# Zejun-Yang/AniPortrait

Measured on NVIDIA H100. Metric: denoised frames/sec @512x512 L=16 steps=25, higher is better.
Workload: dtype fp16

## Files before the change

### aniportrait_b200/csrc/ap_attention.cu

```cuda
#include <stdio.h>
#include <stdlib.h>

#include "ap_host.h"
#include "ap_ptx.cuh"
#include "ap_wgmma.cuh"

namespace ap {

__device__ __forceinline__ float fast_exp2(float x) {
  float y;
  asm("ex2.approx.ftz.f32 %0, %1;" : "=f"(y) : "f"(x));
  return y;
}

struct AttnParams {
  int n_frames, tokens, heads, head_dim;
  int bank_tokens;
  int first_bank_frame;
  int frames_per_bank;
  int m_tiles;
  int num_units;
  float scale_log2;
  __half* out;
  long long ldo;
};

template <int DPAD, int BN>
struct AttnCfg {
  static constexpr int SLABS = DPAD / 64;
  static constexpr int Q_BYTES = 128 * DPAD * 2;
  static constexpr int K_BYTES = BN * DPAD * 2;
  static constexpr int KV_STAGE = 2 * K_BYTES;
  static constexpr int BUDGET = 227 * 1024 - 1024 - 256 - Q_BYTES;
  static constexpr int STAGES_RAW = BUDGET / KV_STAGE;
  static constexpr int STAGES = STAGES_RAW > 4 ? 4 : STAGES_RAW;
  static constexpr int SMEM_BYTES = Q_BYTES + STAGES * KV_STAGE + 1024 + 256;
  static_assert(STAGES >= 2, "need at least a double-buffered K/V ring");
  static_assert(DPAD % 64 == 0 && DPAD <= 192 && (BN == 64 || BN == 128), "tile config");
};

template <int DPAD, int BN>
__global__ void __launch_bounds__(384, 1)
attention_kernel(const __grid_constant__ CUtensorMap tmQ, const __grid_constant__ CUtensorMap tmK,
                 const __grid_constant__ CUtensorMap tmV, const __grid_constant__ CUtensorMap tmBK,
                 const __grid_constant__ CUtensorMap tmBV, const AttnParams p) {
  using Cfg = AttnCfg<DPAD, BN>;
  constexpr int ST = Cfg::STAGES;
  griddep_launch_dependents();
  extern __shared__ uint8_t smem_raw[];
  uint8_t* smem = reinterpret_cast<uint8_t*>((reinterpret_cast<uintptr_t>(smem_raw) + 1023) & ~uintptr_t(1023));
  uint8_t* smem_q = smem;
  uint8_t* smem_kv = smem_q + Cfg::Q_BYTES;
  uint64_t* bars = reinterpret_cast<uint64_t*>(smem_kv + ST * Cfg::KV_STAGE);
  uint64_t* q_full = bars + 0;
  uint64_t* q_empty = bars + 1;
  uint64_t* k_full = bars + 2;
  uint64_t* v_full = k_full + ST;
  uint64_t* kv_empty = v_full + ST;

  const int warp = threadIdx.x >> 5;
  const int lane = threadIdx.x & 31;

  if (warp == 0 && lane == 0) {
    tma_prefetch_desc(&tmQ);
    tma_prefetch_desc(&tmK);
    tma_prefetch_desc(&tmV);
    mbar_init(q_full, 1);
    mbar_init(q_empty, 8);
    for (int s = 0; s < ST; ++s) {
      mbar_init(&k_full[s], 1);
      mbar_init(&v_full[s], 1);
      mbar_init(&kv_empty[s], 8);
    }
    fence_mbar_init();
  }
  __syncthreads();
  griddep_wait();

  const int own_tiles = (p.tokens + BN - 1) / BN;
  const int bank_tiles = (p.bank_tokens + BN - 1) / BN;
  const int units_per_frame = p.heads * p.m_tiles;

  auto decode = [&](int unit, int& frame, int& head, int& m_tile, int& T) {
    const int fk = unit / units_per_frame;
    const int rem = unit % units_per_frame;
    frame = (fk + p.first_bank_frame) % p.n_frames;
    head = rem / p.m_tiles;
    m_tile = rem % p.m_tiles;
    const bool has_bank = p.bank_tokens > 0 && frame >= p.first_bank_frame;
    T = own_tiles + (has_bank ? bank_tiles : 0);
  };

  if (warp < 4) {
    setmaxnreg_dec<40>();
    if (warp == 0 && lane == 0) {
      uint32_t g = 0;
      uint32_t uc = 0;
      for (int unit = blockIdx.x; unit < p.num_units; unit += gridDim.x, ++uc) {
        int frame, head, m_tile, T;
        decode(unit, frame, head, m_tile, T);
        mbar_wait_quiet(q_empty, (uc & 1) ^ 1);
        mbar_arrive_expect_tx(q_full, Cfg::Q_BYTES);
#pragma unroll
        for (int s = 0; s < Cfg::SLABS; ++s)
          tma_load_2d(&tmQ, q_full, smem_q + s * (128 * 128), head * DPAD + s * 64, frame * p.tokens + m_tile * 128);
        const int bank_idx = (frame - p.first_bank_frame) / p.frames_per_bank;
        for (int j = 0; j < T; ++j, ++g) {
          const int stage = g % ST;
          const uint32_t ph = (g / ST) & 1;
          mbar_wait_quiet(&kv_empty[stage], ph ^ 1);
          const bool own = j < own_tiles;
          const CUtensorMap* mk = own ? &tmK : &tmBK;
          const CUtensorMap* mv = own ? &tmV : &tmBV;
          const int row = own ? frame * p.tokens + j * BN : bank_idx * p.bank_tokens + (j - own_tiles) * BN;
          uint8_t* kd = smem_kv + stage * Cfg::KV_STAGE;
          uint8_t* vd = kd + Cfg::K_BYTES;
          mbar_arrive_expect_tx(&k_full[stage], Cfg::K_BYTES);
#pragma unroll
          for (int s = 0; s < Cfg::SLABS; ++s)
            tma_load_2d(mk, &k_full[stage], kd + s * (BN * 128), head * DPAD + s * 64, row);
          mbar_arrive_expect_tx(&v_full[stage], Cfg::K_BYTES);
#pragma unroll
          for (int s = 0; s < Cfg::SLABS; ++s)
            tma_load_2d(mv, &v_full[stage], vd + s * (BN * 128), head * DPAD + s * 64, row);
        }
      }
    }
    return;
  }

  setmaxnreg_inc<232>();
  const int wg = (warp >> 2) - 1;
  const int wq = warp & 3;
  const int qd = lane & 3;
  const uint32_t q_base = smem_u32(smem_q) + wg * (64 * 128);
  uint32_t g = 0, uc = 0;
  for (int unit = blockIdx.x; unit < p.num_units; unit += gridDim.x, ++uc) {
    int frame, head, m_tile, T;
    decode(unit, frame, head, m_tile, T);
    float o[DPAD / 2];
#pragma unroll
    for (int i = 0; i < DPAD / 2; ++i) o[i] = 0.f;
    float m_run[2] = {-INFINITY, -INFINITY}, l_run[2] = {0.f, 0.f};
    mbar_wait_quiet(q_full, uc & 1);
    for (int j = 0; j < T; ++j, ++g) {
      const int stage = g % ST;
      const uint32_t ph = (g / ST) & 1;
      const uint32_t k_addr = smem_u32(smem_kv + stage * Cfg::KV_STAGE);
      const uint32_t v_addr = k_addr + Cfg::K_BYTES;
      float s[BN / 2];
      mbar_wait_quiet(&k_full[stage], ph);
      wgmma_fence();
#pragma unroll
      for (int kk = 0; kk < DPAD / 16; ++kk)
        wgmma_ss<BN>(s, wgmma_desc_k_sw128(q_base + (kk / 4) * (128 * 128) + (kk % 4) * 32),
                     wgmma_desc_k_sw128(k_addr + (kk / 4) * (BN * 128) + (kk % 4) * 32), kk != 0);
      wgmma_commit();
      wgmma_wait<0>();
      reg_fence<BN / 2>(s);
      if (j == T - 1) {
        __syncwarp();
        if (lane == 0) mbar_arrive(q_empty);
      }

      const bool own = j < own_tiles;
      const int jj = own ? j : j - own_tiles;
      const int ntok = own ? p.tokens : p.bank_tokens;
      const int valid = min(BN, ntok - jj * BN);
      if (valid != BN) {
#pragma unroll
        for (int i = 0; i < BN / 8; ++i)
#pragma unroll
          for (int e = 0; e < 2; ++e)
            if (8 * i + 2 * qd + e >= valid) {
              s[4 * i + e] = -INFINITY;
              s[4 * i + 2 + e] = -INFINITY;
            }
      }
      float mx[2] = {s[0], s[2]};
#pragma unroll
      for (int i = 0; i < BN / 8; ++i) {
        mx[0] = fmaxf(mx[0], fmaxf(s[4 * i], s[4 * i + 1]));
        mx[1] = fmaxf(mx[1], fmaxf(s[4 * i + 2], s[4 * i + 3]));
      }
      float alpha[2];
#pragma unroll
      for (int r = 0; r < 2; ++r) {
        mx[r] = fmaxf(mx[r], __shfl_xor_sync(0xffffffffu, mx[r], 1));
        mx[r] = fmaxf(mx[r], __shfl_xor_sync(0xffffffffu, mx[r], 2));
        const float m_new = fmaxf(m_run[r], mx[r] * p.scale_log2);
        alpha[r] = fast_exp2(m_run[r] - m_new);
        m_run[r] = m_new;
        l_run[r] *= alpha[r];
      }
#pragma unroll
      for (int i = 0; i < DPAD / 8; ++i) {
        o[4 * i] *= alpha[0]; o[4 * i + 1] *= alpha[0];
        o[4 * i + 2] *= alpha[1]; o[4 * i + 3] *= alpha[1];
      }
      uint32_t pk[BN / 4];
#pragma unroll
      for (int i = 0; i < BN / 8; ++i) {
        const float p0 = fast_exp2(fmaf(s[4 * i], p.scale_log2, -m_run[0]));
        const float p1 = fast_exp2(fmaf(s[4 * i + 1], p.scale_log2, -m_run[0]));
        const float p2 = fast_exp2(fmaf(s[4 * i + 2], p.scale_log2, -m_run[1]));
        const float p3 = fast_exp2(fmaf(s[4 * i + 3], p.scale_log2, -m_run[1]));
        l_run[0] += p0 + p1;
        l_run[1] += p2 + p3;
        const __half2 h01 = __floats2half2_rn(p0, p1), h23 = __floats2half2_rn(p2, p3);
        pk[2 * i] = *reinterpret_cast<const uint32_t*>(&h01);
        pk[2 * i + 1] = *reinterpret_cast<const uint32_t*>(&h23);
      }
      mbar_wait_quiet(&v_full[stage], ph);
      wgmma_fence();
#pragma unroll
      for (int kk = 0; kk < BN / 16; ++kk)
        wgmma_rs_tb<DPAD>(o, pk + 4 * kk, wgmma_desc_mn_sw128(v_addr + kk * (16 * 128), BN * 128), 1);
      wgmma_commit();
      wgmma_wait<0>();
      reg_fence<DPAD / 2>(o);
      __syncwarp();
      if (lane == 0) mbar_arrive(&kv_empty[stage]);
    }
#pragma unroll
    for (int r = 0; r < 2; ++r) {
      l_run[r] += __shfl_xor_sync(0xffffffffu, l_run[r], 1);
      l_run[r] += __shfl_xor_sync(0xffffffffu, l_run[r], 2);
    }
#pragma unroll
    for (int r = 0; r < 2; ++r) {
      const float inv_l = 1.f / l_run[r];
      const int q_idx = m_tile * 128 + wg * 64 + wq * 16 + (lane >> 2) + 8 * r;
      if (q_idx < p.tokens) {
        __half* dst = p.out + ((long long)frame * p.tokens + q_idx) * p.ldo + head * p.head_dim;
#pragma unroll
        for (int i = 0; i < DPAD / 8; ++i)
          if (8 * i + 2 * qd < p.head_dim)
            *reinterpret_cast<__half2*>(dst + 8 * i + 2 * qd) =
                __floats2half2_rn(o[4 * i + 2 * r] * inv_l, o[4 * i + 2 * r + 1] * inv_l);
      }
    }
  }
}

template <int DPAD, int BN>
static int launch_attention(const CUtensorMap* maps, const AttnParams& p, cudaStream_t stream) {
  using Cfg = AttnCfg<DPAD, BN>;
  static bool attr_set = false;
  if (!attr_set) {
    AP_CHECK_CUDA(cudaFuncSetAttribute(attention_kernel<DPAD, BN>, cudaFuncAttributeMaxDynamicSharedMemorySize,
                                       Cfg::SMEM_BYTES));
    attr_set = true;
  }
  const int grid = p.num_units < num_sms() ? p.num_units : num_sms();
  AP_LAUNCH((attention_kernel<DPAD, BN>), grid, 384, Cfg::SMEM_BYTES, stream, maps[0], maps[1], maps[2], maps[3], maps[4], p);
  AP_CHECK_CUDA(cudaGetLastError());
  return AP_OK;
}

}

using namespace ap;

extern "C" int ap_attention_f16(const void* q, const void* k, const void* v, long long ld_qkv, const void* bank_k,
                                const void* bank_v, long long ld_bank, int bank_tokens, int n_banks, int n_frames,
                                int tokens, int heads, int head_dim, int dpad, int first_bank_frame,
                                int frames_per_bank, float scale, void* out, long long ldo, void* stream) {
  AP_REQUIRE(q && k && v && out, "attention: null pointer");
  AP_REQUIRE(dpad == 64 || dpad == 128 || dpad == 192, "attention: dpad must be 64/128/192 (got %d)", dpad);
  AP_REQUIRE(head_dim % 8 == 0 && head_dim <= dpad, "attention: head_dim %d must be a multiple of 8 and <= dpad", head_dim);
  AP_REQUIRE(ld_qkv % 8 == 0 && ldo % 8 == 0, "attention: leading dims must be multiples of 8 elements");
  AP_REQUIRE((reinterpret_cast<uintptr_t>(out) & 3) == 0, "attention: out must be 4-byte aligned");
  AP_REQUIRE(n_frames > 0 && tokens > 0 && heads > 0, "attention: bad shape");
  const bool has_bank = bank_k != nullptr && bank_tokens > 0;
  AP_REQUIRE(!has_bank || (bank_v && frames_per_bank > 0 && first_bank_frame >= 0 && n_banks > 0),
             "attention: bad bank arguments");
  const int bn = dpad == 192 ? 64 : 128;
  AttnParams p{};
  p.n_frames = n_frames;
  p.tokens = tokens;
  p.heads = heads;
  p.head_dim = head_dim;
  p.bank_tokens = has_bank ? bank_tokens : 0;
  p.first_bank_frame = has_bank ? first_bank_frame : 0;
  p.frames_per_bank = has_bank ? frames_per_bank : 1;
  p.m_tiles = (tokens + 127) / 128;
  p.num_units = n_frames * heads * p.m_tiles;
  p.scale_log2 = scale * 1.4426950408889634f;
  p.out = (__half*)out;
  p.ldo = ldo;
  if (has_bank) {
    const int max_bank = (n_frames - 1 - first_bank_frame) / frames_per_bank;
    AP_REQUIRE(first_bank_frame >= n_frames || max_bank < n_banks, "attention: bank index out of range");
  }

  CUtensorMap maps[5];
  const uint64_t cols = (uint64_t)heads * dpad;
  auto mk = [&](CUtensorMap* tm, const void* base, uint64_t rows, long long ld, uint32_t box_rows) -> int {
    const uint64_t dims[2] = {cols, rows};
    const uint64_t strides[1] = {(uint64_t)ld * 2};
    const uint32_t box[2] = {64, box_rows};
    return encode_tmap(tm, base, 2, dims, strides, box, true);
  };
  int rc;
  const uint64_t rows = (uint64_t)n_frames * tokens;
  if ((rc = mk(&maps[0], q, rows, ld_qkv, 128))) return rc;
  if ((rc = mk(&maps[1], k, rows, ld_qkv, bn))) return rc;
  if ((rc = mk(&maps[2], v, rows, ld_qkv, bn))) return rc;
  if (has_bank) {
    const uint64_t brows = (uint64_t)n_banks * bank_tokens;
    if ((rc = mk(&maps[3], bank_k, brows, ld_bank, bn))) return rc;
    if ((rc = mk(&maps[4], bank_v, brows, ld_bank, bn))) return rc;
  } else {
    maps[3] = maps[1];
    maps[4] = maps[2];
  }
  cudaStream_t st = (cudaStream_t)stream;
  if (dpad == 64) return launch_attention<64, 128>(maps, p, st);
  if (dpad == 128) return launch_attention<128, 128>(maps, p, st);
  return launch_attention<192, 64>(maps, p, st);
}
```

### aniportrait_b200/csrc/ap_ptx.cuh

```cuda
#pragma once
#include <cuda.h>
#include <cuda_fp16.h>
#include <cuda_runtime.h>
#include <stdint.h>
#include <stdio.h>

namespace ap {

__device__ __forceinline__ void griddep_launch_dependents() { asm volatile("griddepcontrol.launch_dependents;" ::: "memory"); }
__device__ __forceinline__ void griddep_wait() { asm volatile("griddepcontrol.wait;" ::: "memory"); }

__device__ __forceinline__ float gelu_erf(float x) {
  const float z = fminf(fabsf(x) * 0.70710678118654752f, 4.3f);
  float q = fmaf(1.686094986e-05f, z, -4.376256625e-04f);
  q = fmaf(q, z, 4.960034474e-03f);
  q = fmaf(q, z, -3.321249048e-02f);
  q = fmaf(q, z, 1.515097036e-01f);
  q = fmaf(q, z, 9.176268788e-01f);
  q = fmaf(q, z, 1.627959694e+00f);
  float e;
  asm("ex2.approx.ftz.f32 %0, %1;" : "=f"(e) : "f"(-q * z));
  return fmaxf(x, 0.f) - z * 0.70710678118654752f * e;
}

__device__ __forceinline__ float quick_gelu(float x) {
  float e, r;
  asm("ex2.approx.ftz.f32 %0, %1;" : "=f"(e) : "f"(x * -2.4554669595930157f));
  asm("rcp.approx.ftz.f32 %0, %1;" : "=f"(r) : "f"(1.f + e));
  return x * r;
}

__device__ __forceinline__ uint32_t smem_u32(const void* p) {
  return static_cast<uint32_t>(__cvta_generic_to_shared(p));
}

__device__ __forceinline__ uint32_t elect_one() {
  uint32_t pred = 0;
  asm volatile(
      "{\n\t"
      ".reg .pred P1;\n\t"
      "elect.sync _|P1, 0xffffffff;\n\t"
      "selp.u32 %0, 1, 0, P1;\n\t"
      "}\n"
      : "=r"(pred));
  return pred;
}

__device__ __forceinline__ void mbar_init(uint64_t* bar, uint32_t count) {
  asm volatile("mbarrier.init.shared::cta.b64 [%0], %1;" ::"r"(smem_u32(bar)), "r"(count) : "memory");
}
__device__ __forceinline__ void fence_mbar_init() {
  asm volatile("fence.mbarrier_init.release.cluster;" ::: "memory");
}
__device__ __forceinline__ void fence_proxy_async_smem() {
  asm volatile("fence.proxy.async.shared::cta;" ::: "memory");
}
__device__ __forceinline__ void mbar_arrive_expect_tx(uint64_t* bar, uint32_t bytes) {
  asm volatile("mbarrier.arrive.expect_tx.shared::cta.b64 _, [%0], %1;" ::"r"(smem_u32(bar)), "r"(bytes)
               : "memory");
}
__device__ __forceinline__ void mbar_arrive(uint64_t* bar) {
  asm volatile("mbarrier.arrive.shared::cta.b64 _, [%0];" ::"r"(smem_u32(bar)) : "memory");
}
__device__ __forceinline__ uint32_t mbar_try_wait(uint64_t* bar, uint32_t parity) {
  uint32_t done;
  asm volatile(
      "{\n\t"
      ".reg .pred P1;\n\t"
      "mbarrier.try_wait.parity.shared::cta.b64 P1, [%1], %2;\n\t"
      "selp.u32 %0, 1, 0, P1;\n\t"
      "}\n"
      : "=r"(done)
      : "r"(smem_u32(bar)), "r"(parity)
      : "memory");
  return done;
}
#ifndef AP_MBAR_TIMEOUT_CYCLES
#define AP_MBAR_TIMEOUT_CYCLES (8000000000ll)
#endif
__device__ __forceinline__ void mbar_wait(uint64_t* bar, uint32_t parity) {
  if (mbar_try_wait(bar, parity)) return;
  long long t0 = clock64();
  while (!mbar_try_wait(bar, parity)) {
    if (clock64() - t0 > AP_MBAR_TIMEOUT_CYCLES) {
      printf("ap: mbarrier timeout block=(%d,%d) thread=%d bar=0x%x parity=%u\n", blockIdx.x, blockIdx.y, threadIdx.x,
             smem_u32(bar), parity);
      __trap();
    }
  }
}

__device__ __forceinline__ void mbar_wait_quiet(uint64_t* bar, uint32_t parity) {
  if (mbar_try_wait(bar, parity)) return;
  long long t0 = clock64();
  while (!mbar_try_wait(bar, parity))
    if (clock64() - t0 > AP_MBAR_TIMEOUT_CYCLES) __trap();
}

__device__ __forceinline__ void tma_prefetch_desc(const CUtensorMap* m) {
  asm volatile("prefetch.tensormap [%0];" ::"l"(reinterpret_cast<uint64_t>(m)) : "memory");
}
__device__ __forceinline__ void tma_load_2d(const CUtensorMap* m, uint64_t* bar, void* dst, int c0, int c1) {
  asm volatile(
      "cp.async.bulk.tensor.2d.shared::cluster.global.mbarrier::complete_tx::bytes [%0], [%1, {%3, %4}], [%2];" ::"r"(
          smem_u32(dst)),
      "l"(reinterpret_cast<uint64_t>(m)), "r"(smem_u32(bar)), "r"(c0), "r"(c1)
      : "memory");
}
__device__ __forceinline__ void tma_load_3d(const CUtensorMap* m, uint64_t* bar, void* dst, int c0, int c1, int c2) {
  asm volatile(
      "cp.async.bulk.tensor.3d.shared::cluster.global.mbarrier::complete_tx::bytes [%0], [%1, {%3, %4, %5}], [%2];" ::
          "r"(smem_u32(dst)),
      "l"(reinterpret_cast<uint64_t>(m)), "r"(smem_u32(bar)), "r"(c0), "r"(c1), "r"(c2)
      : "memory");
}
__device__ __forceinline__ void tma_load_4d(const CUtensorMap* m, uint64_t* bar, void* dst, int c0, int c1, int c2,
                                            int c3) {
  asm volatile(
      "cp.async.bulk.tensor.4d.shared::cluster.global.mbarrier::complete_tx::bytes [%0], [%1, {%3, %4, %5, %6}], "
      "[%2];" ::"r"(smem_u32(dst)),
      "l"(reinterpret_cast<uint64_t>(m)), "r"(smem_u32(bar)), "r"(c0), "r"(c1), "r"(c2), "r"(c3)
      : "memory");
}
__device__ __forceinline__ void tma_load_5d(const CUtensorMap* m, uint64_t* bar, void* dst, int c0, int c1, int c2,
                                            int c3, int c4) {
  asm volatile(
      "cp.async.bulk.tensor.5d.shared::cluster.global.mbarrier::complete_tx::bytes [%0], [%1, {%3, %4, %5, %6, %7}], "
      "[%2];" ::"r"(smem_u32(dst)),
      "l"(reinterpret_cast<uint64_t>(m)), "r"(smem_u32(bar)), "r"(c0), "r"(c1), "r"(c2), "r"(c3), "r"(c4)
      : "memory");
}

__device__ __forceinline__ void tma_store_2d(const CUtensorMap* m, const void* src, int c0, int c1) {
  asm volatile("cp.async.bulk.tensor.2d.global.shared::cta.bulk_group [%0, {%2, %3}], [%1];" ::"l"(
                   reinterpret_cast<uint64_t>(m)),
               "r"(smem_u32(src)), "r"(c0), "r"(c1)
               : "memory");
}
__device__ __forceinline__ void tma_store_4d(const CUtensorMap* m, const void* src, int c0, int c1, int c2, int c3) {
  asm volatile("cp.async.bulk.tensor.4d.global.shared::cta.bulk_group [%0, {%2, %3, %4, %5}], [%1];" ::"l"(
                   reinterpret_cast<uint64_t>(m)),
               "r"(smem_u32(src)), "r"(c0), "r"(c1), "r"(c2), "r"(c3)
               : "memory");
}
__device__ __forceinline__ void tma_store_commit() { asm volatile("cp.async.bulk.commit_group;" ::: "memory"); }
template <int N>
__device__ __forceinline__ void tma_store_wait_read() {
  asm volatile("cp.async.bulk.wait_group.read %0;" ::"n"(N) : "memory");
}
template <int N>
__device__ __forceinline__ void tma_store_wait_all() {
  asm volatile("cp.async.bulk.wait_group %0;" ::"n"(N) : "memory");
}

__device__ __forceinline__ void wgmma_fence() { asm volatile("wgmma.fence.sync.aligned;" ::: "memory"); }
__device__ __forceinline__ void wgmma_commit() { asm volatile("wgmma.commit_group.sync.aligned;" ::: "memory"); }
template <int N>
__device__ __forceinline__ void wgmma_wait() {
  asm volatile("wgmma.wait_group.sync.aligned %0;" ::"n"(N) : "memory");
}
template <int N>
__device__ __forceinline__ void reg_fence(float* r) {
#pragma unroll
  for (int i = 0; i < N; ++i) asm volatile("" : "+f"(r[i])::"memory");
}
template <uint32_t kRegs>
__device__ __forceinline__ void setmaxnreg_inc() { asm volatile("setmaxnreg.inc.sync.aligned.u32 %0;" ::"n"(kRegs)); }
template <uint32_t kRegs>
__device__ __forceinline__ void setmaxnreg_dec() { asm volatile("setmaxnreg.dec.sync.aligned.u32 %0;" ::"n"(kRegs)); }

__device__ __forceinline__ uint64_t wgmma_desc_k_sw128(uint32_t smem_addr) {
  uint64_t d = 0;
  d |= static_cast<uint64_t>((smem_addr >> 4) & 0x3FFF);
  d |= static_cast<uint64_t>(1) << 16;
  d |= static_cast<uint64_t>(1024 >> 4) << 32;
  d |= static_cast<uint64_t>(1) << 62;
  return d;
}
__device__ __forceinline__ uint64_t wgmma_desc_mn_sw128(uint32_t smem_addr, uint32_t lbo_bytes) {
  uint64_t d = 0;
  d |= static_cast<uint64_t>((smem_addr >> 4) & 0x3FFF);
  d |= static_cast<uint64_t>((lbo_bytes >> 4) & 0x3FFF) << 16;
  d |= static_cast<uint64_t>(1024 >> 4) << 32;
  d |= static_cast<uint64_t>(1) << 62;
  return d;
}

__device__ __forceinline__ void named_bar_sync(uint32_t id, uint32_t nthreads) {
  asm volatile("bar.sync %0, %1;" ::"r"(id), "r"(nthreads) : "memory");
}

}
```

### aniportrait_b200/csrc/ap_wgmma.cuh

```cuda
#pragma once
#include <stdint.h>

namespace ap {

template <int N>
__device__ __forceinline__ void wgmma_ss(float* d, uint64_t da, uint64_t db, uint32_t scale_d);
template <int N>
__device__ __forceinline__ void wgmma_rs_tb(float* d, const uint32_t* a, uint64_t db, uint32_t scale_d);

template <>
__device__ __forceinline__ void wgmma_ss<32>(float* d, uint64_t da, uint64_t db, uint32_t scale_d) {
  asm volatile(
      "{\n\t.reg .pred p;\n\tsetp.ne.b32 p, %18, 0;\n\t"
      "wgmma.mma_async.sync.aligned.m64n32k16.f32.f16.f16 {%0, %1, %2, %3, %4, %5, %6, %7, %8, %9, %10, %11, %12, %13, %14, %15}, %16, %17, p, 1, 1, 0, 0;\n\t}\n"
      : "+f"(d[0]), "+f"(d[1]), "+f"(d[2]), "+f"(d[3]), "+f"(d[4]), "+f"(d[5]), "+f"(d[6]), "+f"(d[7]), "+f"(d[8]), "+f"(d[9]), "+f"(d[10]), "+f"(d[11]), "+f"(d[12]), "+f"(d[13]), "+f"(d[14]), "+f"(d[15])
      : "l"(da), "l"(db), "r"(scale_d));
}
template <>
__device__ __forceinline__ void wgmma_ss<64>(float* d, uint64_t da, uint64_t db, uint32_t scale_d) {
  asm volatile(
      "{\n\t.reg .pred p;\n\tsetp.ne.b32 p, %34, 0;\n\t"
      "wgmma.mma_async.sync.aligned.m64n64k16.f32.f16.f16 {%0, %1, %2, %3, %4, %5, %6, %7, %8, %9, %10, %11, %12, %13, %14, %15, %16, %17, %18, %19, %20, %21, %22, %23, %24, %25, %26, %27, %28, %29, %30, %31}, %32, %33, p, 1, 1, 0, 0;\n\t}\n"
      : "+f"(d[0]), "+f"(d[1]), "+f"(d[2]), "+f"(d[3]), "+f"(d[4]), "+f"(d[5]), "+f"(d[6]), "+f"(d[7]), "+f"(d[8]), "+f"(d[9]), "+f"(d[10]), "+f"(d[11]), "+f"(d[12]), "+f"(d[13]), "+f"(d[14]), "+f"(d[15]), "+f"(d[16]), "+f"(d[17]), "+f"(d[18]), "+f"(d[19]), "+f"(d[20]), "+f"(d[21]), "+f"(d[22]), "+f"(d[23]), "+f"(d[24]), "+f"(d[25]), "+f"(d[26]), "+f"(d[27]), "+f"(d[28]), "+f"(d[29]), "+f"(d[30]), "+f"(d[31])
      : "l"(da), "l"(db), "r"(scale_d));
}
template <>
__device__ __forceinline__ void wgmma_ss<128>(float* d, uint64_t da, uint64_t db, uint32_t scale_d) {
  asm volatile(
      "{\n\t.reg .pred p;\n\tsetp.ne.b32 p, %66, 0;\n\t"
      "wgmma.mma_async.sync.aligned.m64n128k16.f32.f16.f16 {%0, %1, %2, %3, %4, %5, %6, %7, %8, %9, %10, %11, %12, %13, %14, %15, %16, %17, %18, %19, %20, %21, %22, %23, %24, %25, %26, %27, %28, %29, %30, %31, %32, %33, %34, %35, %36, %37, %38, %39, %40, %41, %42, %43, %44, %45, %46, %47, %48, %49, %50, %51, %52, %53, %54, %55, %56, %57, %58, %59, %60, %61, %62, %63}, %64, %65, p, 1, 1, 0, 0;\n\t}\n"
      : "+f"(d[0]), "+f"(d[1]), "+f"(d[2]), "+f"(d[3]), "+f"(d[4]), "+f"(d[5]), "+f"(d[6]), "+f"(d[7]), "+f"(d[8]), "+f"(d[9]), "+f"(d[10]), "+f"(d[11]), "+f"(d[12]), "+f"(d[13]), "+f"(d[14]), "+f"(d[15]), "+f"(d[16]), "+f"(d[17]), "+f"(d[18]), "+f"(d[19]), "+f"(d[20]), "+f"(d[21]), "+f"(d[22]), "+f"(d[23]), "+f"(d[24]), "+f"(d[25]), "+f"(d[26]), "+f"(d[27]), "+f"(d[28]), "+f"(d[29]), "+f"(d[30]), "+f"(d[31]), "+f"(d[32]), "+f"(d[33]), "+f"(d[34]), "+f"(d[35]), "+f"(d[36]), "+f"(d[37]), "+f"(d[38]), "+f"(d[39]), "+f"(d[40]), "+f"(d[41]), "+f"(d[42]), "+f"(d[43]), "+f"(d[44]), "+f"(d[45]), "+f"(d[46]), "+f"(d[47]), "+f"(d[48]), "+f"(d[49]), "+f"(d[50]), "+f"(d[51]), "+f"(d[52]), "+f"(d[53]), "+f"(d[54]), "+f"(d[55]), "+f"(d[56]), "+f"(d[57]), "+f"(d[58]), "+f"(d[59]), "+f"(d[60]), "+f"(d[61]), "+f"(d[62]), "+f"(d[63])
      : "l"(da), "l"(db), "r"(scale_d));
}
template <>
__device__ __forceinline__ void wgmma_ss<160>(float* d, uint64_t da, uint64_t db, uint32_t scale_d) {
  asm volatile(
      "{\n\t.reg .pred p;\n\tsetp.ne.b32 p, %82, 0;\n\t"
      "wgmma.mma_async.sync.aligned.m64n160k16.f32.f16.f16 {%0, %1, %2, %3, %4, %5, %6, %7, %8, %9, %10, %11, %12, %13, %14, %15, %16, %17, %18, %19, %20, %21, %22, %23, %24, %25, %26, %27, %28, %29, %30, %31, %32, %33, %34, %35, %36, %37, %38, %39, %40, %41, %42, %43, %44, %45, %46, %47, %48, %49, %50, %51, %52, %53, %54, %55, %56, %57, %58, %59, %60, %61, %62, %63, %64, %65, %66, %67, %68, %69, %70, %71, %72, %73, %74, %75, %76, %77, %78, %79}, %80, %81, p, 1, 1, 0, 0;\n\t}\n"
      : "+f"(d[0]), "+f"(d[1]), "+f"(d[2]), "+f"(d[3]), "+f"(d[4]), "+f"(d[5]), "+f"(d[6]), "+f"(d[7]), "+f"(d[8]), "+f"(d[9]), "+f"(d[10]), "+f"(d[11]), "+f"(d[12]), "+f"(d[13]), "+f"(d[14]), "+f"(d[15]), "+f"(d[16]), "+f"(d[17]), "+f"(d[18]), "+f"(d[19]), "+f"(d[20]), "+f"(d[21]), "+f"(d[22]), "+f"(d[23]), "+f"(d[24]), "+f"(d[25]), "+f"(d[26]), "+f"(d[27]), "+f"(d[28]), "+f"(d[29]), "+f"(d[30]), "+f"(d[31]), "+f"(d[32]), "+f"(d[33]), "+f"(d[34]), "+f"(d[35]), "+f"(d[36]), "+f"(d[37]), "+f"(d[38]), "+f"(d[39]), "+f"(d[40]), "+f"(d[41]), "+f"(d[42]), "+f"(d[43]), "+f"(d[44]), "+f"(d[45]), "+f"(d[46]), "+f"(d[47]), "+f"(d[48]), "+f"(d[49]), "+f"(d[50]), "+f"(d[51]), "+f"(d[52]), "+f"(d[53]), "+f"(d[54]), "+f"(d[55]), "+f"(d[56]), "+f"(d[57]), "+f"(d[58]), "+f"(d[59]), "+f"(d[60]), "+f"(d[61]), "+f"(d[62]), "+f"(d[63]), "+f"(d[64]), "+f"(d[65]), "+f"(d[66]), "+f"(d[67]), "+f"(d[68]), "+f"(d[69]), "+f"(d[70]), "+f"(d[71]), "+f"(d[72]), "+f"(d[73]), "+f"(d[74]), "+f"(d[75]), "+f"(d[76]), "+f"(d[77]), "+f"(d[78]), "+f"(d[79])
      : "l"(da), "l"(db), "r"(scale_d));
}
template <>
__device__ __forceinline__ void wgmma_ss<256>(float* d, uint64_t da, uint64_t db, uint32_t scale_d) {
  asm volatile(
      "{\n\t.reg .pred p;\n\tsetp.ne.b32 p, %130, 0;\n\t"
      "wgmma.mma_async.sync.aligned.m64n256k16.f32.f16.f16 {%0, %1, %2, %3, %4, %5, %6, %7, %8, %9, %10, %11, %12, %13, %14, %15, %16, %17, %18, %19, %20, %21, %22, %23, %24, %25, %26, %27, %28, %29, %30, %31, %32, %33, %34, %35, %36, %37, %38, %39, %40, %41, %42, %43, %44, %45, %46, %47, %48, %49, %50, %51, %52, %53, %54, %55, %56, %57, %58, %59, %60, %61, %62, %63, %64, %65, %66, %67, %68, %69, %70, %71, %72, %73, %74, %75, %76, %77, %78, %79, %80, %81, %82, %83, %84, %85, %86, %87, %88, %89, %90, %91, %92, %93, %94, %95, %96, %97, %98, %99, %100, %101, %102, %103, %104, %105, %106, %107, %108, %109, %110, %111, %112, %113, %114, %115, %116, %117, %118, %119, %120, %121, %122, %123, %124, %125, %126, %127}, %128, %129, p, 1, 1, 0, 0;\n\t}\n"
      : "+f"(d[0]), "+f"(d[1]), "+f"(d[2]), "+f"(d[3]), "+f"(d[4]), "+f"(d[5]), "+f"(d[6]), "+f"(d[7]), "+f"(d[8]), "+f"(d[9]), "+f"(d[10]), "+f"(d[11]), "+f"(d[12]), "+f"(d[13]), "+f"(d[14]), "+f"(d[15]), "+f"(d[16]), "+f"(d[17]), "+f"(d[18]), "+f"(d[19]), "+f"(d[20]), "+f"(d[21]), "+f"(d[22]), "+f"(d[23]), "+f"(d[24]), "+f"(d[25]), "+f"(d[26]), "+f"(d[27]), "+f"(d[28]), "+f"(d[29]), "+f"(d[30]), "+f"(d[31]), "+f"(d[32]), "+f"(d[33]), "+f"(d[34]), "+f"(d[35]), "+f"(d[36]), "+f"(d[37]), "+f"(d[38]), "+f"(d[39]), "+f"(d[40]), "+f"(d[41]), "+f"(d[42]), "+f"(d[43]), "+f"(d[44]), "+f"(d[45]), "+f"(d[46]), "+f"(d[47]), "+f"(d[48]), "+f"(d[49]), "+f"(d[50]), "+f"(d[51]), "+f"(d[52]), "+f"(d[53]), "+f"(d[54]), "+f"(d[55]), "+f"(d[56]), "+f"(d[57]), "+f"(d[58]), "+f"(d[59]), "+f"(d[60]), "+f"(d[61]), "+f"(d[62]), "+f"(d[63]), "+f"(d[64]), "+f"(d[65]), "+f"(d[66]), "+f"(d[67]), "+f"(d[68]), "+f"(d[69]), "+f"(d[70]), "+f"(d[71]), "+f"(d[72]), "+f"(d[73]), "+f"(d[74]), "+f"(d[75]), "+f"(d[76]), "+f"(d[77]), "+f"(d[78]), "+f"(d[79]), "+f"(d[80]), "+f"(d[81]), "+f"(d[82]), "+f"(d[83]), "+f"(d[84]), "+f"(d[85]), "+f"(d[86]), "+f"(d[87]), "+f"(d[88]), "+f"(d[89]), "+f"(d[90]), "+f"(d[91]), "+f"(d[92]), "+f"(d[93]), "+f"(d[94]), "+f"(d[95]), "+f"(d[96]), "+f"(d[97]), "+f"(d[98]), "+f"(d[99]), "+f"(d[100]), "+f"(d[101]), "+f"(d[102]), "+f"(d[103]), "+f"(d[104]), "+f"(d[105]), "+f"(d[106]), "+f"(d[107]), "+f"(d[108]), "+f"(d[109]), "+f"(d[110]), "+f"(d[111]), "+f"(d[112]), "+f"(d[113]), "+f"(d[114]), "+f"(d[115]), "+f"(d[116]), "+f"(d[117]), "+f"(d[118]), "+f"(d[119]), "+f"(d[120]), "+f"(d[121]), "+f"(d[122]), "+f"(d[123]), "+f"(d[124]), "+f"(d[125]), "+f"(d[126]), "+f"(d[127])
      : "l"(da), "l"(db), "r"(scale_d));
}
template <>
__device__ __forceinline__ void wgmma_rs_tb<64>(float* d, const uint32_t* a, uint64_t db, uint32_t scale_d) {
  asm volatile(
      "{\n\t.reg .pred p;\n\tsetp.ne.b32 p, %37, 0;\n\t"
      "wgmma.mma_async.sync.aligned.m64n64k16.f32.f16.f16 {%0, %1, %2, %3, %4, %5, %6, %7, %8, %9, %10, %11, %12, %13, %14, %15, %16, %17, %18, %19, %20, %21, %22, %23, %24, %25, %26, %27, %28, %29, %30, %31}, {%32, %33, %34, %35}, %36, p, 1, 1, 1;\n\t}\n"
      : "+f"(d[0]), "+f"(d[1]), "+f"(d[2]), "+f"(d[3]), "+f"(d[4]), "+f"(d[5]), "+f"(d[6]), "+f"(d[7]), "+f"(d[8]), "+f"(d[9]), "+f"(d[10]), "+f"(d[11]), "+f"(d[12]), "+f"(d[13]), "+f"(d[14]), "+f"(d[15]), "+f"(d[16]), "+f"(d[17]), "+f"(d[18]), "+f"(d[19]), "+f"(d[20]), "+f"(d[21]), "+f"(d[22]), "+f"(d[23]), "+f"(d[24]), "+f"(d[25]), "+f"(d[26]), "+f"(d[27]), "+f"(d[28]), "+f"(d[29]), "+f"(d[30]), "+f"(d[31])
      : "r"(a[0]), "r"(a[1]), "r"(a[2]), "r"(a[3]), "l"(db), "r"(scale_d));
}
template <>
__device__ __forceinline__ void wgmma_rs_tb<128>(float* d, const uint32_t* a, uint64_t db, uint32_t scale_d) {
  asm volatile(
      "{\n\t.reg .pred p;\n\tsetp.ne.b32 p, %69, 0;\n\t"
      "wgmma.mma_async.sync.aligned.m64n128k16.f32.f16.f16 {%0, %1, %2, %3, %4, %5, %6, %7, %8, %9, %10, %11, %12, %13, %14, %15, %16, %17, %18, %19, %20, %21, %22, %23, %24, %25, %26, %27, %28, %29, %30, %31, %32, %33, %34, %35, %36, %37, %38, %39, %40, %41, %42, %43, %44, %45, %46, %47, %48, %49, %50, %51, %52, %53, %54, %55, %56, %57, %58, %59, %60, %61, %62, %63}, {%64, %65, %66, %67}, %68, p, 1, 1, 1;\n\t}\n"
      : "+f"(d[0]), "+f"(d[1]), "+f"(d[2]), "+f"(d[3]), "+f"(d[4]), "+f"(d[5]), "+f"(d[6]), "+f"(d[7]), "+f"(d[8]), "+f"(d[9]), "+f"(d[10]), "+f"(d[11]), "+f"(d[12]), "+f"(d[13]), "+f"(d[14]), "+f"(d[15]), "+f"(d[16]), "+f"(d[17]), "+f"(d[18]), "+f"(d[19]), "+f"(d[20]), "+f"(d[21]), "+f"(d[22]), "+f"(d[23]), "+f"(d[24]), "+f"(d[25]), "+f"(d[26]), "+f"(d[27]), "+f"(d[28]), "+f"(d[29]), "+f"(d[30]), "+f"(d[31]), "+f"(d[32]), "+f"(d[33]), "+f"(d[34]), "+f"(d[35]), "+f"(d[36]), "+f"(d[37]), "+f"(d[38]), "+f"(d[39]), "+f"(d[40]), "+f"(d[41]), "+f"(d[42]), "+f"(d[43]), "+f"(d[44]), "+f"(d[45]), "+f"(d[46]), "+f"(d[47]), "+f"(d[48]), "+f"(d[49]), "+f"(d[50]), "+f"(d[51]), "+f"(d[52]), "+f"(d[53]), "+f"(d[54]), "+f"(d[55]), "+f"(d[56]), "+f"(d[57]), "+f"(d[58]), "+f"(d[59]), "+f"(d[60]), "+f"(d[61]), "+f"(d[62]), "+f"(d[63])
      : "r"(a[0]), "r"(a[1]), "r"(a[2]), "r"(a[3]), "l"(db), "r"(scale_d));
}
template <>
__device__ __forceinline__ void wgmma_rs_tb<192>(float* d, const uint32_t* a, uint64_t db, uint32_t scale_d) {
  asm volatile(
      "{\n\t.reg .pred p;\n\tsetp.ne.b32 p, %101, 0;\n\t"
      "wgmma.mma_async.sync.aligned.m64n192k16.f32.f16.f16 {%0, %1, %2, %3, %4, %5, %6, %7, %8, %9, %10, %11, %12, %13, %14, %15, %16, %17, %18, %19, %20, %21, %22, %23, %24, %25, %26, %27, %28, %29, %30, %31, %32, %33, %34, %35, %36, %37, %38, %39, %40, %41, %42, %43, %44, %45, %46, %47, %48, %49, %50, %51, %52, %53, %54, %55, %56, %57, %58, %59, %60, %61, %62, %63, %64, %65, %66, %67, %68, %69, %70, %71, %72, %73, %74, %75, %76, %77, %78, %79, %80, %81, %82, %83, %84, %85, %86, %87, %88, %89, %90, %91, %92, %93, %94, %95}, {%96, %97, %98, %99}, %100, p, 1, 1, 1;\n\t}\n"
      : "+f"(d[0]), "+f"(d[1]), "+f"(d[2]), "+f"(d[3]), "+f"(d[4]), "+f"(d[5]), "+f"(d[6]), "+f"(d[7]), "+f"(d[8]), "+f"(d[9]), "+f"(d[10]), "+f"(d[11]), "+f"(d[12]), "+f"(d[13]), "+f"(d[14]), "+f"(d[15]), "+f"(d[16]), "+f"(d[17]), "+f"(d[18]), "+f"(d[19]), "+f"(d[20]), "+f"(d[21]), "+f"(d[22]), "+f"(d[23]), "+f"(d[24]), "+f"(d[25]), "+f"(d[26]), "+f"(d[27]), "+f"(d[28]), "+f"(d[29]), "+f"(d[30]), "+f"(d[31]), "+f"(d[32]), "+f"(d[33]), "+f"(d[34]), "+f"(d[35]), "+f"(d[36]), "+f"(d[37]), "+f"(d[38]), "+f"(d[39]), "+f"(d[40]), "+f"(d[41]), "+f"(d[42]), "+f"(d[43]), "+f"(d[44]), "+f"(d[45]), "+f"(d[46]), "+f"(d[47]), "+f"(d[48]), "+f"(d[49]), "+f"(d[50]), "+f"(d[51]), "+f"(d[52]), "+f"(d[53]), "+f"(d[54]), "+f"(d[55]), "+f"(d[56]), "+f"(d[57]), "+f"(d[58]), "+f"(d[59]), "+f"(d[60]), "+f"(d[61]), "+f"(d[62]), "+f"(d[63]), "+f"(d[64]), "+f"(d[65]), "+f"(d[66]), "+f"(d[67]), "+f"(d[68]), "+f"(d[69]), "+f"(d[70]), "+f"(d[71]), "+f"(d[72]), "+f"(d[73]), "+f"(d[74]), "+f"(d[75]), "+f"(d[76]), "+f"(d[77]), "+f"(d[78]), "+f"(d[79]), "+f"(d[80]), "+f"(d[81]), "+f"(d[82]), "+f"(d[83]), "+f"(d[84]), "+f"(d[85]), "+f"(d[86]), "+f"(d[87]), "+f"(d[88]), "+f"(d[89]), "+f"(d[90]), "+f"(d[91]), "+f"(d[92]), "+f"(d[93]), "+f"(d[94]), "+f"(d[95])
      : "r"(a[0]), "r"(a[1]), "r"(a[2]), "r"(a[3]), "l"(db), "r"(scale_d));
}

}
```

Before: 5.681.

## Ping-pong warpgroups, overlap PV with next QK, trim MMA width to head dim

The two consumer warpgroups now take turns issuing tensor-core work through named barriers, so one warpgroup's softmax overlaps the other's MMAs. Within each warpgroup, the P·V MMA for tile j and the Q·K MMA for tile j+1 go out in a single batch, which cuts wgmma wait points. The P·V output width and the QK k-steps are templated on the real head dim (40/80/88/160), so the padded columns are no longer computed. The row-max uses a tree reduction, and the K/V ring may grow to 6 stages. In exchange, the barrier bookkeeping for the last unit and for T==1 is more intricate, and there is a deadlock or correctness risk if the turn barriers fall out of sync.

Measured after the change: 5.724 (median of 6 runs). About the same (+0.8%).

```diff
diff --git a/aniportrait_b200/csrc/ap_attention.cu b/aniportrait_b200/csrc/ap_attention.cu
--- a/aniportrait_b200/csrc/ap_attention.cu
+++ b/aniportrait_b200/csrc/ap_attention.cu
@@ -33,19 +33,21 @@
   static constexpr int KV_STAGE = 2 * K_BYTES;
   static constexpr int BUDGET = 227 * 1024 - 1024 - 256 - Q_BYTES;
   static constexpr int STAGES_RAW = BUDGET / KV_STAGE;
-  static constexpr int STAGES = STAGES_RAW > 4 ? 4 : STAGES_RAW;
+  static constexpr int STAGES = STAGES_RAW > 6 ? 6 : STAGES_RAW;
   static constexpr int SMEM_BYTES = Q_BYTES + STAGES * KV_STAGE + 1024 + 256;
   static_assert(STAGES >= 2, "need at least a double-buffered K/V ring");
   static_assert(DPAD % 64 == 0 && DPAD <= 192 && (BN == 64 || BN == 128), "tile config");
 };
 
-template <int DPAD, int BN>
+template <int DPAD, int BN, int NV>
 __global__ void __launch_bounds__(384, 1)
 attention_kernel(const __grid_constant__ CUtensorMap tmQ, const __grid_constant__ CUtensorMap tmK,
                  const __grid_constant__ CUtensorMap tmV, const __grid_constant__ CUtensorMap tmBK,
                  const __grid_constant__ CUtensorMap tmBV, const AttnParams p) {
   using Cfg = AttnCfg<DPAD, BN>;
   constexpr int ST = Cfg::STAGES;
+  constexpr int KSTEPS = (NV + 15) / 16;
+  static_assert(NV % 8 == 0 && NV <= DPAD, "MMA width");
   griddep_launch_dependents();
   extern __shared__ uint8_t smem_raw[];
   uint8_t* smem = reinterpret_cast<uint8_t*>((reinterpret_cast<uintptr_t>(smem_raw) + 1023) & ~uintptr_t(1023));
@@ -134,35 +136,42 @@
   const int wq = warp & 3;
   const int qd = lane & 3;
   const uint32_t q_base = smem_u32(smem_q) + wg * (64 * 128);
+  constexpr uint32_t TURN_BAR = 1;
+  if (wg == 1) named_bar_arrive(TURN_BAR + 0, 256);
   uint32_t g = 0, uc = 0;
   for (int unit = blockIdx.x; unit < p.num_units; unit += gridDim.x, ++uc) {
     int frame, head, m_tile, T;
     decode(unit, frame, head, m_tile, T);
-    float o[DPAD / 2];
-#pragma unroll
-    for (int i = 0; i < DPAD / 2; ++i) o[i] = 0.f;
+    const bool last_unit = unit + (int)gridDim.x >= p.num_units;
+    float o[NV / 2];
+#pragma unroll
+    for (int i = 0; i < NV / 2; ++i) o[i] = 0.f;
     float m_run[2] = {-INFINITY, -INFINITY}, l_run[2] = {0.f, 0.f};
-    mbar_wait_quiet(q_full, uc & 1);
-    for (int j = 0; j < T; ++j, ++g) {
-      const int stage = g % ST;
-      const uint32_t ph = (g / ST) & 1;
-      const uint32_t k_addr = smem_u32(smem_kv + stage * Cfg::KV_STAGE);
-      const uint32_t v_addr = k_addr + Cfg::K_BYTES;
-      float s[BN / 2];
-      mbar_wait_quiet(&k_full[stage], ph);
-      wgmma_fence();
-#pragma unroll
-      for (int kk = 0; kk < DPAD / 16; ++kk)
+    float s[BN / 2];
+    uint32_t pk[BN / 4];
+    auto issue_s = [&](uint32_t gs) {
+      const uint32_t k_addr = smem_u32(smem_kv + (gs % ST) * Cfg::KV_STAGE);
+#pragma unroll
+      for (int kk = 0; kk < KSTEPS; ++kk)
         wgmma_ss<BN>(s, wgmma_desc_k_sw128(q_base + (kk / 4) * (128 * 128) + (kk % 4) * 32),
                      wgmma_desc_k_sw128(k_addr + (kk / 4) * (BN * 128) + (kk % 4) * 32), kk != 0);
-      wgmma_commit();
-      wgmma_wait<0>();
-      reg_fence<BN / 2>(s);
-      if (j == T - 1) {
-        __syncwarp();
-        if (lane == 0) mbar_arrive(q_empty);
-      }
-
+    };
+    auto issue_pv = [&](uint32_t gs) {
+      const uint32_t v_addr = smem_u32(smem_kv + (gs % ST) * Cfg::KV_STAGE) + Cfg::K_BYTES;
+#pragma unroll
+      for (int kk = 0; kk < BN / 16; ++kk)
+        wgmma_rs_tb<NV>(o, pk + 4 * kk, wgmma_desc_mn_sw128(v_addr + kk * (16 * 128), BN * 128), 1);
+    };
+    mbar_wait_quiet(q_full, uc & 1);
+    mbar_wait_quiet(&k_full[g % ST], (g / ST) & 1);
+    named_bar_sync(TURN_BAR + wg, 256);
+    wgmma_fence();
+    issue_s(g);
+    wgmma_commit();
+    named_bar_arrive(TURN_BAR + (wg ^ 1), 256);
+    wgmma_wait<0>();
+    reg_fence<BN / 2>(s);
+    for (int j = 0;; ++j, ++g) {
       const bool own = j < own_tiles;
       const int jj = own ? j : j - own_tiles;
       const int ntok = own ? p.tokens : p.bank_tokens;
@@ -177,12 +186,21 @@
               s[4 * i + 2 + e] = -INFINITY;
             }
       }
-      float mx[2] = {s[0], s[2]};
+      float t0[BN / 8], t1[BN / 8];
 #pragma unroll
       for (int i = 0; i < BN / 8; ++i) {
-        mx[0] = fmaxf(mx[0], fmaxf(s[4 * i], s[4 * i + 1]));
-        mx[1] = fmaxf(mx[1], fmaxf(s[4 * i + 2], s[4 * i + 3]));
-      }
+        t0[i] = fmaxf(s[4 * i], s[4 * i + 1]);
+        t1[i] = fmaxf(s[4 * i + 2], s[4 * i + 3]);
+      }
+#pragma unroll
+      for (int w = BN / 16; w >= 1; w >>= 1)
+#pragma unroll
+        for (int i = 0; i < BN / 16; ++i)
+          if (i < w) {
+            t0[i] = fmaxf(t0[i], t0[i + w]);
+            t1[i] = fmaxf(t1[i], t1[i + w]);
+          }
+      float mx[2] = {t0[0], t1[0]};
       float alpha[2];
 #pragma unroll
       for (int r = 0; r < 2; ++r) {
@@ -194,11 +212,10 @@
         l_run[r] *= alpha[r];
       }
 #pragma unroll
-      for (int i = 0; i < DPAD / 8; ++i) {
+      for (int i = 0; i < NV / 8; ++i) {
         o[4 * i] *= alpha[0]; o[4 * i + 1] *= alpha[0];
         o[4 * i + 2] *= alpha[1]; o[4 * i + 3] *= alpha[1];
       }
-      uint32_t pk[BN / 4];
 #pragma unroll
       for (int i = 0; i < BN / 8; ++i) {
         const float p0 = fast_exp2(fmaf(s[4 * i], p.scale_log2, -m_run[0]));
@@ -211,17 +228,35 @@
         pk[2 * i] = *reinterpret_cast<const uint32_t*>(&h01);
         pk[2 * i + 1] = *reinterpret_cast<const uint32_t*>(&h23);
       }
-      mbar_wait_quiet(&v_full[stage], ph);
+      mbar_wait_quiet(&v_full[g % ST], (g / ST) & 1);
+      if (j + 1 == T) break;
+      mbar_wait_quiet(&k_full[(g + 1) % ST], ((g + 1) / ST) & 1);
+      named_bar_sync(TURN_BAR + wg, 256);
       wgmma_fence();
-#pragma unroll
-      for (int kk = 0; kk < BN / 16; ++kk)
-        wgmma_rs_tb<DPAD>(o, pk + 4 * kk, wgmma_desc_mn_sw128(v_addr + kk * (16 * 128), BN * 128), 1);
+      issue_pv(g);
+      issue_s(g + 1);
       wgmma_commit();
+      named_bar_arrive(TURN_BAR + (wg ^ 1), 256);
       wgmma_wait<0>();
-      reg_fence<DPAD / 2>(o);
+      reg_fence<NV / 2>(o);
+      reg_fence<BN / 2>(s);
       __syncwarp();
-      if (lane == 0) mbar_arrive(&kv_empty[stage]);
-    }
+      if (lane == 0) {
+        mbar_arrive(&kv_empty[g % ST]);
+        if (j + 2 == T) mbar_arrive(q_empty);
+      }
+    }
+    if (T == 1 && lane == 0) mbar_arrive(q_empty);
+    named_bar_sync(TURN_BAR + wg, 256);
+    wgmma_fence();
+    issue_pv(g);
+    wgmma_commit();
+    if (!last_unit || wg == 0) named_bar_arrive(TURN_BAR + (wg ^ 1), 256);
+    wgmma_wait<0>();
+    reg_fence<NV / 2>(o);
+    __syncwarp();
+    if (lane == 0) mbar_arrive(&kv_empty[g % ST]);
+    ++g;
 #pragma unroll
     for (int r = 0; r < 2; ++r) {
       l_run[r] += __shfl_xor_sync(0xffffffffu, l_run[r], 1);
@@ -234,7 +269,7 @@
       if (q_idx < p.tokens) {
         __half* dst = p.out + ((long long)frame * p.tokens + q_idx) * p.ldo + head * p.head_dim;
 #pragma unroll
-        for (int i = 0; i < DPAD / 8; ++i)
+        for (int i = 0; i < NV / 8; ++i)
           if (8 * i + 2 * qd < p.head_dim)
             *reinterpret_cast<__half2*>(dst + 8 * i + 2 * qd) =
                 __floats2half2_rn(o[4 * i + 2 * r] * inv_l, o[4 * i + 2 * r + 1] * inv_l);
@@ -243,17 +278,18 @@
   }
 }
 
-template <int DPAD, int BN>
+template <int DPAD, int BN, int NV>
 static int launch_attention(const CUtensorMap* maps, const AttnParams& p, cudaStream_t stream) {
   using Cfg = AttnCfg<DPAD, BN>;
   static bool attr_set = false;
   if (!attr_set) {
-    AP_CHECK_CUDA(cudaFuncSetAttribute(attention_kernel<DPAD, BN>, cudaFuncAttributeMaxDynamicSharedMemorySize,
+    AP_CHECK_CUDA(cudaFuncSetAttribute(attention_kernel<DPAD, BN, NV>, cudaFuncAttributeMaxDynamicSharedMemorySize,
                                        Cfg::SMEM_BYTES));
     attr_set = true;
   }
   const int grid = p.num_units < num_sms() ? p.num_units : num_sms();
-  AP_LAUNCH((attention_kernel<DPAD, BN>), grid, 384, Cfg::SMEM_BYTES, stream, maps[0], maps[1], maps[2], maps[3], maps[4], p);
+  AP_LAUNCH((attention_kernel<DPAD, BN, NV>), grid, 384, Cfg::SMEM_BYTES, stream, maps[0], maps[1], maps[2], maps[3], maps[4],
+            p);
   AP_CHECK_CUDA(cudaGetLastError());
   return AP_OK;
 }
@@ -316,7 +352,11 @@
     maps[4] = maps[2];
   }
   cudaStream_t st = (cudaStream_t)stream;
-  if (dpad == 64) return launch_attention<64, 128>(maps, p, st);
-  if (dpad == 128) return launch_attention<128, 128>(maps, p, st);
-  return launch_attention<192, 64>(maps, p, st);
-}
+  if (dpad == 64) return head_dim == 40 ? launch_attention<64, 128, 40>(maps, p, st) : launch_attention<64, 128, 64>(maps, p, st);
+  if (dpad == 128) {
+    if (head_dim == 80) return launch_attention<128, 128, 80>(maps, p, st);
+    if (head_dim == 88) return launch_attention<128, 128, 88>(maps, p, st);
+    return launch_attention<128, 128, 128>(maps, p, st);
+  }
+  return head_dim == 160 ? launch_attention<192, 64, 160>(maps, p, st) : launch_attention<192, 64, 192>(maps, p, st);
+}
diff --git a/aniportrait_b200/csrc/ap_ptx.cuh b/aniportrait_b200/csrc/ap_ptx.cuh
--- a/aniportrait_b200/csrc/ap_ptx.cuh
+++ b/aniportrait_b200/csrc/ap_ptx.cuh
@@ -189,5 +189,8 @@
 __device__ __forceinline__ void named_bar_sync(uint32_t id, uint32_t nthreads) {
   asm volatile("bar.sync %0, %1;" ::"r"(id), "r"(nthreads) : "memory");
 }
+__device__ __forceinline__ void named_bar_arrive(uint32_t id, uint32_t nthreads) {
+  asm volatile("bar.arrive %0, %1;" ::"r"(id), "r"(nthreads) : "memory");
+}
 
 }
diff --git a/aniportrait_b200/csrc/ap_wgmma.cuh b/aniportrait_b200/csrc/ap_wgmma.cuh
--- a/aniportrait_b200/csrc/ap_wgmma.cuh
+++ b/aniportrait_b200/csrc/ap_wgmma.cuh
@@ -49,6 +49,14 @@
       : "l"(da), "l"(db), "r"(scale_d));
 }
 template <>
+__device__ __forceinline__ void wgmma_rs_tb<40>(float* d, const uint32_t* a, uint64_t db, uint32_t scale_d) {
+  asm volatile(
+      "{\n\t.reg .pred p;\n\tsetp.ne.b32 p, %25, 0;\n\t"
+      "wgmma.mma_async.sync.aligned.m64n40k16.f32.f16.f16 {%0, %1, %2, %3, %4, %5, %6, %7, %8, %9, %10, %11, %12, %13, %14, %15, %16, %17, %18, %19}, {%20, %21, %22, %23}, %24, p, 1, 1, 1;\n\t}\n"
+      : "+f"(d[0]), "+f"(d[1]), "+f"(d[2]), "+f"(d[3]), "+f"(d[4]), "+f"(d[5]), "+f"(d[6]), "+f"(d[7]), "+f"(d[8]), "+f"(d[9]), "+f"(d[10]), "+f"(d[11]), "+f"(d[12]), "+f"(d[13]), "+f"(d[14]), "+f"(d[15]), "+f"(d[16]), "+f"(d[17]), "+f"(d[18]), "+f"(d[19])
+      : "r"(a[0]), "r"(a[1]), "r"(a[2]), "r"(a[3]), "l"(db), "r"(scale_d));
+}
+template <>
 __device__ __forceinline__ void wgmma_rs_tb<64>(float* d, const uint32_t* a, uint64_t db, uint32_t scale_d) {
   asm volatile(
       "{\n\t.reg .pred p;\n\tsetp.ne.b32 p, %37, 0;\n\t"
@@ -57,11 +65,35 @@
       : "r"(a[0]), "r"(a[1]), "r"(a[2]), "r"(a[3]), "l"(db), "r"(scale_d));
 }
 template <>
+__device__ __forceinline__ void wgmma_rs_tb<80>(float* d, const uint32_t* a, uint64_t db, uint32_t scale_d) {
+  asm volatile(
+      "{\n\t.reg .pred p;\n\tsetp.ne.b32 p, %45, 0;\n\t"
+      "wgmma.mma_async.sync.aligned.m64n80k16.f32.f16.f16 {%0, %1, %2, %3, %4, %5, %6, %7, %8, %9, %10, %11, %12, %13, %14, %15, %16, %17, %18, %19, %20, %21, %22, %23, %24, %25, %26, %27, %28, %29, %30, %31, %32, %33, %34, %35, %36, %37, %38, %39}, {%40, %41, %42, %43}, %44, p, 1, 1, 1;\n\t}\n"
+      : "+f"(d[0]), "+f"(d[1]), "+f"(d[2]), "+f"(d[3]), "+f"(d[4]), "+f"(d[5]), "+f"(d[6]), "+f"(d[7]), "+f"(d[8]), "+f"(d[9]), "+f"(d[10]), "+f"(d[11]), "+f"(d[12]), "+f"(d[13]), "+f"(d[14]), "+f"(d[15]), "+f"(d[16]), "+f"(d[17]), "+f"(d[18]), "+f"(d[19]), "+f"(d[20]), "+f"(d[21]), "+f"(d[22]), "+f"(d[23]), "+f"(d[24]), "+f"(d[25]), "+f"(d[26]), "+f"(d[27]), "+f"(d[28]), "+f"(d[29]), "+f"(d[30]), "+f"(d[31]), "+f"(d[32]), "+f"(d[33]), "+f"(d[34]), "+f"(d[35]), "+f"(d[36]), "+f"(d[37]), "+f"(d[38]), "+f"(d[39])
+      : "r"(a[0]), "r"(a[1]), "r"(a[2]), "r"(a[3]), "l"(db), "r"(scale_d));
+}
+template <>
+__device__ __forceinline__ void wgmma_rs_tb<88>(float* d, const uint32_t* a, uint64_t db, uint32_t scale_d) {
+  asm volatile(
+      "{\n\t.reg .pred p;\n\tsetp.ne.b32 p, %49, 0;\n\t"
+      "wgmma.mma_async.sync.aligned.m64n88k16.f32.f16.f16 {%0, %1, %2, %3, %4, %5, %6, %7, %8, %9, %10, %11, %12, %13, %14, %15, %16, %17, %18, %19, %20, %21, %22, %23, %24, %25, %26, %27, %28, %29, %30, %31, %32, %33, %34, %35, %36, %37, %38, %39, %40, %41, %42, %43}, {%44, %45, %46, %47}, %48, p, 1, 1, 1;\n\t}\n"
+      : "+f"(d[0]), "+f"(d[1]), "+f"(d[2]), "+f"(d[3]), "+f"(d[4]), "+f"(d[5]), "+f"(d[6]), "+f"(d[7]), "+f"(d[8]), "+f"(d[9]), "+f"(d[10]), "+f"(d[11]), "+f"(d[12]), "+f"(d[13]), "+f"(d[14]), "+f"(d[15]), "+f"(d[16]), "+f"(d[17]), "+f"(d[18]), "+f"(d[19]), "+f"(d[20]), "+f"(d[21]), "+f"(d[22]), "+f"(d[23]), "+f"(d[24]), "+f"(d[25]), "+f"(d[26]), "+f"(d[27]), "+f"(d[28]), "+f"(d[29]), "+f"(d[30]), "+f"(d[31]), "+f"(d[32]), "+f"(d[33]), "+f"(d[34]), "+f"(d[35]), "+f"(d[36]), "+f"(d[37]), "+f"(d[38]), "+f"(d[39]), "+f"(d[40]), "+f"(d[41]), "+f"(d[42]), "+f"(d[43])
+      : "r"(a[0]), "r"(a[1]), "r"(a[2]), "r"(a[3]), "l"(db), "r"(scale_d));
+}
+template <>
 __device__ __forceinline__ void wgmma_rs_tb<128>(float* d, const uint32_t* a, uint64_t db, uint32_t scale_d) {
   asm volatile(
       "{\n\t.reg .pred p;\n\tsetp.ne.b32 p, %69, 0;\n\t"
       "wgmma.mma_async.sync.aligned.m64n128k16.f32.f16.f16 {%0, %1, %2, %3, %4, %5, %6, %7, %8, %9, %10, %11, %12, %13, %14, %15, %16, %17, %18, %19, %20, %21, %22, %23, %24, %25, %26, %27, %28, %29, %30, %31, %32, %33, %34, %35, %36, %37, %38, %39, %40, %41, %42, %43, %44, %45, %46, %47, %48, %49, %50, %51, %52, %53, %54, %55, %56, %57, %58, %59, %60, %61, %62, %63}, {%64, %65, %66, %67}, %68, p, 1, 1, 1;\n\t}\n"
       : "+f"(d[0]), "+f"(d[1]), "+f"(d[2]), "+f"(d[3]), "+f"(d[4]), "+f"(d[5]), "+f"(d[6]), "+f"(d[7]), "+f"(d[8]), "+f"(d[9]), "+f"(d[10]), "+f"(d[11]), "+f"(d[12]), "+f"(d[13]), "+f"(d[14]), "+f"(d[15]), "+f"(d[16]), "+f"(d[17]), "+f"(d[18]), "+f"(d[19]), "+f"(d[20]), "+f"(d[21]), "+f"(d[22]), "+f"(d[23]), "+f"(d[24]), "+f"(d[25]), "+f"(d[26]), "+f"(d[27]), "+f"(d[28]), "+f"(d[29]), "+f"(d[30]), "+f"(d[31]), "+f"(d[32]), "+f"(d[33]), "+f"(d[34]), "+f"(d[35]), "+f"(d[36]), "+f"(d[37]), "+f"(d[38]), "+f"(d[39]), "+f"(d[40]), "+f"(d[41]), "+f"(d[42]), "+f"(d[43]), "+f"(d[44]), "+f"(d[45]), "+f"(d[46]), "+f"(d[47]), "+f"(d[48]), "+f"(d[49]), "+f"(d[50]), "+f"(d[51]), "+f"(d[52]), "+f"(d[53]), "+f"(d[54]), "+f"(d[55]), "+f"(d[56]), "+f"(d[57]), "+f"(d[58]), "+f"(d[59]), "+f"(d[60]), "+f"(d[61]), "+f"(d[62]), "+f"(d[63])
+      : "r"(a[0]), "r"(a[1]), "r"(a[2]), "r"(a[3]), "l"(db), "r"(scale_d));
+}
+template <>
+__device__ __forceinline__ void wgmma_rs_tb<160>(float* d, const uint32_t* a, uint64_t db, uint32_t scale_d) {
+  asm volatile(
+      "{\n\t.reg .pred p;\n\tsetp.ne.b32 p, %85, 0;\n\t"
+      "wgmma.mma_async.sync.aligned.m64n160k16.f32.f16.f16 {%0, %1, %2, %3, %4, %5, %6, %7, %8, %9, %10, %11, %12, %13, %14, %15, %16, %17, %18, %19, %20, %21, %22, %23, %24, %25, %26, %27, %28, %29, %30, %31, %32, %33, %34, %35, %36, %37, %38, %39, %40, %41, %42, %43, %44, %45, %46, %47, %48, %49, %50, %51, %52, %53, %54, %55, %56, %57, %58, %59, %60, %61, %62, %63, %64, %65, %66, %67, %68, %69, %70, %71, %72, %73, %74, %75, %76, %77, %78, %79}, {%80, %81, %82, %83}, %84, p, 1, 1, 1;\n\t}\n"
+      : "+f"(d[0]), "+f"(d[1]), "+f"(d[2]), "+f"(d[3]), "+f"(d[4]), "+f"(d[5]), "+f"(d[6]), "+f"(d[7]), "+f"(d[8]), "+f"(d[9]), "+f"(d[10]), "+f"(d[11]), "+f"(d[12]), "+f"(d[13]), "+f"(d[14]), "+f"(d[15]), "+f"(d[16]), "+f"(d[17]), "+f"(d[18]), "+f"(d[19]), "+f"(d[20]), "+f"(d[21]), "+f"(d[22]), "+f"(d[23]), "+f"(d[24]), "+f"(d[25]), "+f"(d[26]), "+f"(d[27]), "+f"(d[28]), "+f"(d[29]), "+f"(d[30]), "+f"(d[31]), "+f"(d[32]), "+f"(d[33]), "+f"(d[34]), "+f"(d[35]), "+f"(d[36]), "+f"(d[37]), "+f"(d[38]), "+f"(d[39]), "+f"(d[40]), "+f"(d[41]), "+f"(d[42]), "+f"(d[43]), "+f"(d[44]), "+f"(d[45]), "+f"(d[46]), "+f"(d[47]), "+f"(d[48]), "+f"(d[49]), "+f"(d[50]), "+f"(d[51]), "+f"(d[52]), "+f"(d[53]), "+f"(d[54]), "+f"(d[55]), "+f"(d[56]), "+f"(d[57]), "+f"(d[58]), "+f"(d[59]), "+f"(d[60]), "+f"(d[61]), "+f"(d[62]), "+f"(d[63]), "+f"(d[64]), "+f"(d[65]), "+f"(d[66]), "+f"(d[67]), "+f"(d[68]), "+f"(d[69]), "+f"(d[70]), "+f"(d[71]), "+f"(d[72]), "+f"(d[73]), "+f"(d[74]), "+f"(d[75]), "+f"(d[76]), "+f"(d[77]), "+f"(d[78]), "+f"(d[79])
       : "r"(a[0]), "r"(a[1]), "r"(a[2]), "r"(a[3]), "l"(db), "r"(scale_d));
 }
 template <>
```
